# fgcallari/skeres

Measured on AMD Instinct MI355X. Metric: LM iterations/sec, higher is better.
Workload: dtype f64

## Files before the change

skeres_amd/csrc/capi.hip:

```cpp
#include <cmath>
#include <cstdlib>
#include <new>

#include "bal_kernels.hpp"
#include "dense_kernels.hpp"
#include "dense_rows_kernels.hpp"
#include "evaluate_kernels.hpp"
#include "cgnr_plan.hpp"
#include "covariance.hpp"
#include "evaluate_plan.hpp"
#include "solver.hpp"

using namespace sk;

struct sk_ptrvec { std::vector<double*> v; };
struct sk_loss_function { LossFunction l; };
struct sk_cost_function { CostFunction c; };
struct sk_problem { Problem p; };
struct sk_local_parameterization { LocalParameterization p; };
struct sk_options { Options o; };
struct sk_summary { Summary s; };
struct sk_solver { std::unique_ptr<SolverBase> impl; };
struct sk_covariance_options { CovarianceOptions o; };
struct sk_covariance { Covariance c; explicit sk_covariance(const CovarianceOptions& o) : c(o) {} };
// ... 40 lines not shown
    if (const char* e = getenv("SK_DEBUG")) {
      const std::string topics = std::string(",") + e + ",";
      k.debug_queues = topics.find(",queues,") != std::string::npos;
      k.debug_envelope = topics.find(",envelope,") != std::string::npos;
      k.debug_segments = topics.find(",segments,") != std::string::npos;
      k.debug_setup = topics.find(",setup,") != std::string::npos;
      k.debug_chain_abort = topics.find(",chain_abort,") != std::string::npos;
    }
    k.queue_shift = num("SK_QUEUE_SHIFT", 0);
    k.chain_queues = num("SK_CHAIN_QUEUES", -1);
    k.pair_max_trailing = num("SK_CHAIN_PAIR_MAX_TRAILING", 0);
    k.dissect_at = num("SK_DISSECT_AT", -1);
    k.schedule_plain = num("SK_SCHEDULE_PLAIN", 0);
    k.cgnr_batch = num("SK_CGNR_BATCH", 0);
    k.chain_xcd_local = num("SK_CHAIN_XCD_LOCAL", 0);
    if (const char* e = getenv("SK_BS_PAIR")) k.bs_pair = atoi(e);
    if (const char* e = getenv("SK_BS_SPREAD")) k.bs_spread = atoi(e);
    if (const char* e = getenv("SK_CHAIN_EARLY_SERVER")) k.chain_early_server = atoi(e);
    if (const char* e = getenv("SK_BULK_RESERVE")) {
      k.bulk_reserve = atoi(e);
      const char* c = strchr(e, ',');
      k.bulk_reserve_early = c ? atoi(c + 1) : k.bulk_reserve;
    }
    return k;
  }();
  return knobs;
}
}

extern "C" {
// ... 1186 lines not shown
```

skeres_amd/csrc/chol_kernels.hip:

```cpp
#include <hip/hip_runtime.h>
#include <algorithm>
#include <atomic>
#include <chrono>
#include <hip/hip_ext.h>
#include <math.h>
#include <stdlib.h>
#include <string.h>
#include <memory>
#include "chol_kernels.hpp"
#include "device_table.hpp"

namespace sk {

typedef double d4 __attribute__((ext_vector_type(4)));

constexpr int gemm_lds_doubles(int kBKT, int kTM, int kTN) { return 2 * (kTM + kTN) * (kBKT + 2); }
#define SK_GEMM_LDS(kBKT, kTM, kTN) __shared__ __attribute__((aligned(16))) double sh[gemm_lds_doubles(kBKT, kTM, kTN)];
template <int kMode, int kShape, int kBKT, int kPF, int kTM, int kTN>
__device__ __forceinline__ void gemm_nt_f64_body(double* shp, double* C, long ldc, const double* A, long lda, const double* B, long ldb, int K,
                                                 int tiles_m, int skip, int main_t = 0x7fffffff, int jump_t = 0, int main_n = 0x7fffffff,
                                                 int jump_n = 0, int block_id = -1, int* first_column_done = nullptr, int count_cols = 1,
                                                 int* diag_done = nullptr) {
  constexpr int mode = kMode;
  constexpr int kLdT = kBKT + 2;
// ... 376 lines not shown
#pragma unroll
    for (int nt = 0; nt < 2; ++nt)
#pragma unroll
      for (int i = 0; i < 4; ++i) acc[mt][nt][i] = sgn * src[(mt * 16 + l4 + 4 * i) * kBs + nt * 16 + l15];
}
__device__ __forceinline__ void block_update32(double* Cb, const double* P, const double* Q, int lane) {
  d4 acc[2][2];
  block_load32(acc, Cb, lane, -1.0);
  block_mma32<false>(acc, P, Q, lane);
  block_store32(Cb, acc, lane, -1.0);
}
__device__ __forceinline__ void block_to_global(double* dst, unsigned step2, unsigned goff, const double* src, int loff) {
#pragma unroll
  for (int i = 0; i < 16; ++i) dst[goff + i * step2] = src[loff + i * 2 * kBs];
}
__device__ __forceinline__ void block_neg_left_mul32(double* dst, const double* W, int lane) {
  d4 acc[2][2];
  block_zero32(acc);
  block_mma32<true>(acc, W, dst, lane);
  block_store32(dst, acc, lane, -1.0);
}

#ifdef SK_POTRF_STAMPS
__device__ long long g_potrf_stamps[4][16], g_potrf_clk[4][16];
#define SK_STAMP(i) if (lane == 0) { g_potrf_stamps[wave][i] = wall_clock64(); g_potrf_clk[wave][i] = clock64(); }
#else
#define SK_STAMP(i)
#endif

__device__ __forceinline__ void info_raise(int* info, int v) { (void)__hip_atomic_fetch_max(info, v, __ATOMIC_RELAXED, __HIP_MEMORY_SCOPE_AGENT); }

__device__ __forceinline__ void potrf128_body(double* lds_in, double* __restrict__ A, long ld, double* __restrict__ Linv, int* info) {
  double* lds = lds_in;
  int tid = threadIdx.x;
  asm volatile("" : "+v"(tid), "+s"(ld));
  double* T = lds;
  double* E = lds + 16 * kBlk;
  double* colbuf = lds + 18 * kBlk;
  volatile int* flags = reinterpret_cast<volatile int*>(colbuf + 192);
  const int t = tid, lane = t & 63, wave = __builtin_amdgcn_readfirstlane(t >> 6);
  __builtin_amdgcn_s_setprio(3);
  SK_STAMP(0)
  {
    double v0[4];
#pragma unroll
    for (int i = 0; i < 4; ++i) {
      const int e = t + 256 * i;
      v0[i] = A[(long)(e >> 5) * ld + (e & 31)];
    }
    if (wave == 0) {
#pragma unroll
      for (int i = 0; i < 4; ++i) { const int e = t + 256 * i; T[blk_off(0, 0) + (e >> 5) * kBs + (e & 31)] = v0[i]; }
      if (t < 4) flags[t] = 0;
      __syncthreads();
    } else {
      double v[3][16];
      const int first = 3 * (wave - 1) + 1;
      const long lo = (long)(lane >> 5) * ld + (lane & 31);
#pragma unroll
      for (int k = 0; k < 3; ++k) {
        const int idx = first + k, bi = idx >= 6 ? 3 : (idx >= 3 ? 2 : 1), bj = idx - bi * (bi + 1) / 2;
        const double* Ab = A + ((long)bi * kB * ld + bj * kB) + lo;
#pragma unroll
        for (int i = 0; i < 16; ++i) v[k][i] = Ab[(long)(2 * i) * ld];
      }
#pragma unroll
      for (int i = 0; i < 4; ++i) { const int e = t + 256 * i; T[blk_off(0, 0) + (e >> 5) * kBs + (e & 31)] = v0[i]; }
      __syncthreads();
// ... 26 lines not shown
    d4 xq;                                                                                       \
    quad_mma16(xq, SK_L((jb) + 1, jb), SK_L(jb, jb), qi, qj, lane, true);                        \
    __syncthreads();                                         \
    quad_store16(SK_L((jb) + 1, jb), xq, qi, qj, lane, 1.0);                                     \
    __syncthreads();                                                 \
    d4 uq;                                                                                       \
    quad_load16(uq, SK_L((jb) + 1, (jb) + 1), qi, qj, lane, -1.0);                               \
    quad_mma16(uq, SK_L((jb) + 1, jb), SK_L((jb) + 1, jb), qi, qj, lane, false);                 \
    quad_store16(SK_L((jb) + 1, (jb) + 1), uq, qi, qj, lane, -1.0);                              \
    __syncthreads();                                                                             \
  }
#define SK_WRITE_L(bi, bj) block_to_global(SK_GA(bi, bj), 2 * uld, go_a, SK_L(bi, bj), lo_w);
#define SK_WRITE_W(bi) block_to_global(SK_GI(bi, bi), 256u, go_i, SK_L(bi, bi), lo_w);
#define SK_WRITE_V(bi, bj) block_to_global(SK_GI(bi, bj), 256u, go_i, SK_V(bi, bj), lo_w);
#define SK_WRITE_E(bi) block_to_global(SK_GA(bi, bi), 2 * uld, go_a, E + ((bi) & 1) * kBlk, lo_w);
#define SK_FLAG_SET(i) { __builtin_amdgcn_fence(__ATOMIC_RELEASE, "workgroup"); __builtin_amdgcn_wave_barrier(); if (lane == 0) flags[i] = 1; }
#define SK_FLAG_WAIT(i) { while (__builtin_amdgcn_readfirstlane(flags[i]) == 0) __builtin_amdgcn_s_sleep(1); __builtin_amdgcn_fence(__ATOMIC_ACQUIRE, "workgroup"); }
  const int qi = wave >> 1, qj = wave & 1;
  if (wave == 0) {
#pragma unroll 1
    for (int jb = 0; jb < 4; ++jb) {
      double* D = SK_L(jb, jb);
      double a[32];
      const bool ok = wave_potrf32(D, colbuf, a, lane);
      SK_STAMP(11 + jb)
      if (!ok && lane == 0) info_raise(info, 1);
      {
        const int row = lane & 31;
        double* dst = lane < 32 ? E + (jb & 1) * kBlk + row * kBs : D + row;
        const int step = lane < 32 ? 1 : kBs;
// ... 6 lines not shown
      if (jb == 1) SK_CRITICAL_B(1)
      if (jb == 2) SK_CRITICAL_B(2)
      SK_STAMP(3 + 2 * jb)
    }
  } else {
    d4 accs[2][2];
    SK_STAMP(2)
    __syncthreads();
    SK_CRITICAL_B(0)
    SK_STAMP(3)
    if (wave == 1) {
      SK_PANEL_ROW(0, 2)
      SK_FLAG_SET(0)
      block_update32(SK_L(2, 2), SK_L(2, 0), SK_L(2, 0), lane);
      block_update32(SK_L(2, 1), SK_L(2, 0), SK_L(1, 0), lane);
      SK_WRITE_L(2, 0)
    }
    if (wave == 2) {
      SK_PANEL_ROW(0, 3)
      SK_FLAG_SET(1)
      block_update32(SK_L(3, 3), SK_L(3, 0), SK_L(3, 0), lane);
      block_update32(SK_L(3, 1), SK_L(3, 0), SK_L(1, 0), lane);
      SK_WRITE_L(3, 0)
    }
    if (wave == 3) {
      SK_WRITE_E(0) SK_WRITE_L(1, 0) SK_WRITE_W(0)
      SK_FLAG_WAIT(0) SK_FLAG_WAIT(1)
      block_update32(SK_L(3, 2), SK_L(3, 0), SK_L(2, 0), lane);
    }
    SK_STAMP(4)
    __syncthreads();
    SK_CRITICAL_B(1)
    SK_STAMP(5)
    if (wave == 1) {
      SK_PANEL_ROW(1, 3)
      block_update32(SK_L(3, 3), SK_L(3, 1), SK_L(3, 1), lane);
      block_update32(SK_L(3, 2), SK_L(3, 1), SK_L(2, 1), lane);
      SK_WRITE_L(3, 1) SK_WRITE_L(2, 1)
    }
    if (wave == 2) {
      d4 acc[2][2];
      block_zero32(acc);
      block_mma32<true>(acc, SK_L(1, 0), SK_L(0, 0), lane);
      block_store32(SK_V(1, 0), acc, lane, 1.0);
      block_neg_left_mul32(SK_V(1, 0), SK_L(1, 1), lane);
      SK_FLAG_SET(2)
      block_zero32(acc);
      block_mma32<true>(acc, SK_L(2, 1), SK_L(1, 1), lane);
      block_store32(SK_V(2, 1), acc, lane, 1.0);
      SK_WRITE_V(1, 0)
    }
    if (wave == 3) {
      SK_WRITE_E(1) SK_WRITE_W(1)
      block_zero32(accs);
      block_mma32<true>(accs, SK_L(2, 0), SK_L(0, 0), lane);
      SK_FLAG_WAIT(2)
      block_mma32<true>(accs, SK_L(2, 1), SK_V(1, 0), lane);
      block_store32(SK_V(2, 0), accs, lane, 1.0);
    }
    SK_STAMP(6)
    __syncthreads();
    SK_CRITICAL_B(2)
    SK_STAMP(7)
    if (wave == 1) {
      block_zero32(accs);
      block_mma32<true>(accs, SK_L(3, 0), SK_L(0, 0), lane);
      block_mma32<true>(accs, SK_L(3, 1), SK_V(1, 0), lane);
      SK_WRITE_L(3, 2)
      SK_FLAG_WAIT(3)
      block_mma32<true>(accs, SK_L(3, 2), SK_V(2, 0), lane);
      block_store32(SK_V(3, 0), accs, lane, 1.0);
      SK_WRITE_V(2, 0)
    }
    if (wave == 2) {
      block_neg_left_mul32(SK_V(2, 1), SK_L(2, 2), lane);
      block_zero32(accs);
      block_mma32<true>(accs, SK_L(3, 1), SK_L(1, 1), lane);
      block_mma32<true>(accs, SK_L(3, 2), SK_V(2, 1), lane);
      block_store32(SK_V(3, 1), accs, lane, 1.0);
      SK_WRITE_V(2, 1)
    }
    if (wave == 3) {
      block_neg_left_mul32(SK_V(2, 0), SK_L(2, 2), lane);
      SK_FLAG_SET(3)
      block_zero32(accs);
      block_mma32<true>(accs, SK_L(3, 2), SK_L(2, 2), lane);
      block_store32(SK_V(3, 2), accs, lane, 1.0);
      SK_WRITE_E(2) SK_WRITE_W(2)
    }
    SK_STAMP(8)
    __syncthreads();
  }
  if (wave < 3) {
    block_neg_left_mul32(SK_V(3, wave), SK_L(3, 3), lane);
    SK_WRITE_V(3, wave)
  } else {
    SK_WRITE_E(3) SK_WRITE_W(3)
  }
  SK_STAMP(10)
#undef SK_PANEL_ROW
#undef SK_CRITICAL_B
#undef SK_FLAG_SET
#undef SK_FLAG_WAIT
#undef SK_WRITE_L
#undef SK_WRITE_W
#undef SK_WRITE_V
#undef SK_WRITE_E
#undef SK_L
#undef SK_V
#undef SK_GA
#undef SK_GI
}

__global__ __launch_bounds__(256, 1) void potrf128_kernel(double* __restrict__ A, long ld, double* __restrict__ Linv, int* info) {
  extern __shared__ __attribute__((aligned(16))) double lds[];
  potrf128_body(lds, A, ld, Linv, info);
}
enum : int { kSyncPotrfDone = 0, kSyncAbort = 1, kSyncSyrkSeq = 2, kSyncSyrkColumn = 3, kSyncServerXcc = 4, kSyncPotrfFast = 5, kSyncStart = 6, kSyncEnd = 7,
             kSyncXSlot = 16, kSyncDSlot = 32, kSyncHeader = 64 };
constexpr int kSyncArrays = 3;
constexpr int kCritCandidates = 160;
constexpr long long kChainTimeoutTicks = 100000000;

__device__ long long g_chain_stamps[1024][8];
__device__ int g_chain_stamps_on;
#define SK_CHAIN_STAMP(col, i) if (g_chain_stamps_on && threadIdx.x == 0 && (col) < 512) g_chain_stamps[(col) + 512 * stamp_front][i] = wall_clock64();
__device__ __forceinline__ int sync_load(const int* p) { return __hip_atomic_load(p, __ATOMIC_RELAXED, __HIP_MEMORY_SCOPE_AGENT); }
__device__ __forceinline__ bool chain_wait(const int* p, int target, int* abort_flag) {
  if (sync_load(p) < target) {
    const long long t0 = wall_clock64();
    do {
      __builtin_amdgcn_s_sleep(4);
      if (sync_load(abort_flag) != 0) return false;
      if (wall_clock64() - t0 > kChainTimeoutTicks) {
        __hip_atomic_store(abort_flag, 1, __ATOMIC_RELAXED, __HIP_MEMORY_SCOPE_AGENT);
        return false;
      }
    } while (sync_load(p) < target);
  }
  __builtin_amdgcn_fence(__ATOMIC_ACQUIRE, "agent");
  asm volatile("s_waitcnt vmcnt(0)" ::: "memory");
  return true;
}
__device__ __forceinline__ bool chain_wait_start(const int* p, int value) {
  if (sync_load(p) != value) {
    const long long t0 = wall_clock64();
    int spins = 0;
    do {
      __builtin_amdgcn_s_sleep(8);
      if ((++spins & 63) == 0 && wall_clock64() - t0 > 30 * kChainTimeoutTicks) return false;
    } while (sync_load(p) != value);
  }
  __builtin_amdgcn_fence(__ATOMIC_ACQUIRE, "agent");
  asm volatile("s_waitcnt vmcnt(0)" ::: "memory");
  return true;
}
#ifdef SK_CHAIN_STRONG_FENCES
// ... 133 lines not shown
    __syncthreads();
  }
  if (local && threadIdx.x == 0) __hip_atomic_store(sync + kSyncServerXcc, 1 + xcc_id(), __ATOMIC_RELAXED, __HIP_MEMORY_SCOPE_AGENT);
  for (int r = 0; r < ranges.n; ++r)
    for (int j = ranges.begin[r]; j < ranges.end[r]; ++j) {
      if (j > 0) {
        if (threadIdx.x == 0) ok_s = server_wait_diag(sync, j, local) ? 1 : 0;
        __syncthreads();
        if (!ok_s) {
          if (threadIdx.x == 0) info_raise(info, 2);
          return;
        }
        SK_CHAIN_ACQUIRE_ALL
      }
      SK_CHAIN_STAMP(j, 0)
      potrf128_body(lds, S + (long)j * 128 * ld + (long)j * 128, ld, Linv + (long)j * 128 * 128, info);
      if (local) {
        asm volatile("s_waitcnt vmcnt(0) lgkmcnt(0)" ::: "memory");
        __syncthreads();
        if (threadIdx.x == 0) {
          store_l2(sync + kSyncPotrfFast, j + 1);
          SK_CHAIN_STAMP(j, 1)
          __builtin_amdgcn_fence(__ATOMIC_RELEASE, "agent");
          __hip_atomic_fetch_add(sync + kSyncPotrfDone, j + 1 - done, __ATOMIC_RELAXED, __HIP_MEMORY_SCOPE_AGENT);
        }
      } else {
        chain_publish(sync + kSyncPotrfDone, j + 1 - done);
        SK_CHAIN_STAMP(j, 1)
      }
      done = j + 1;
    }
// ... 42 lines not shown
  d4 acc1 = {0.0, 0.0, 0.0, 0.0};
#pragma unroll
  for (int kk = 0; kk < 32; kk += 2) {
    acc = __builtin_amdgcn_mfma_f64_16x16x4f64(sa[kk * 4], sb[kk * 4], acc, 0, 0, 0);
    acc1 = __builtin_amdgcn_mfma_f64_16x16x4f64(sa[kk * 4 + 4], sb[kk * 4 + 4], acc1, 0, 0, 0);
  }
  return acc + acc1;
}
__device__ __forceinline__ long crit_tile_off(long ldc, int i) {
  const int lane = threadIdx.x & 63, wave = threadIdx.x >> 6;
  return (long)((wave >> 1) * 16 + (lane >> 4) + 4 * i) * ldc + (wave & 1) * 16 + (lane & 15);
}

__device__ __forceinline__ void chain_column_body(int b, double* S, long ld, int j, const double* Linv_j, int tiles_m, int main_t, int jump_t,
                                                  int ncrit, double* Xs, int* sync, int maxblk, int syrk_need, int column_need, int* info, int do_next, int wait_first,
                                                  int ncand) {
  __shared__ __attribute__((aligned(16))) double sh[2 * 32 * kCritLd];
  static_assert(2 * 32 * kCritLd >= gemm_lds_doubles(16, 32, 128), "LDS of the thin tiles");
  __shared__ int ok_s;
  const int stamp_front = gridDim.y == 2 ? (int)blockIdx.y : 0;
  __builtin_amdgcn_s_setprio(2);
  double* A21 = S + (long)(j + 1) * 128 * ld + (long)j * 128;
  int* x_ready = sync + kSyncHeader + maxblk + j;
  int* diag_ready = sync + kSyncHeader + j + 1;
  int* abort_flag = sync + kSyncAbort;
  const bool local = ncand > ncrit;
  bool crit = b < ncand;
  if (crit && local) {
    if (threadIdx.x == 0) {
      int t = -1;
      if (chain_wait(sync + kSyncServerXcc, 1, abort_flag) && sync_load(sync + kSyncServerXcc) == 1 + xcc_id())
// ... 89 lines not shown
        for (int i = 0; i < 8; ++i) *reinterpret_cast<double2*>(sh + (32 + row) * kCritLd + c0 + 2 * i) = vb[i];
      }
    }
    __syncthreads();
    if (lower) {
      cacc = crit_tile_mma(sh, cacc);
#pragma unroll
      for (int i = 0; i < 4; ++i) Ct[crit_tile_off(ld, i)] = -cacc[i];
    }
    asm volatile("s_waitcnt vmcnt(0) lgkmcnt(0)" ::: "memory");
    __syncthreads();
    if (threadIdx.x == 0) store_l2(sync + kSyncDSlot + b, j + 1);
    if (stamp) SK_CHAIN_STAMP(j, 6)
    return;
  }
  if (threadIdx.x == 0)
    ok_s = (chain_wait(sync + kSyncPotrfDone, j + 1, abort_flag) &&
            (!wait_first || (chain_wait(sync + kSyncSyrkSeq, syrk_need, abort_flag) && chain_wait(sync + kSyncSyrkColumn, column_need, abort_flag)))) ? 1 : 0;
  __syncthreads();
  if (!ok_s) { if (threadIdx.x == 0) info_raise(info, 2); return; }
  SK_CHAIN_ACQUIRE_ALL
  if (stamp) SK_CHAIN_STAMP(j, 3)
  d4 xacc = {0.0, 0.0, 0.0, 0.0};
  if (crit) {
    crit_tile_load(sh, A21 + (long)ri * 32 * ld, ld, Linv_j + (long)q * 32 * 128, 128);
    __syncthreads();
    xacc = crit_tile_mma(sh, xacc);
#pragma unroll
    for (int i = 0; i < 4; ++i) store_through(Xs + (long)(ri * 32) * 128 + q * 32 + crit_tile_off(128, i), xacc[i]);
    chain_publish_through(x_ready, 1);
  } else {
    gemm_nt_f64_body<1, 0, 16, 2, 32, 128>(sh, A21, ld, A21, ld, Linv_j, 128, 128, tiles_m, 0, main_t, jump_t, 0x7fffffff, 0, thin_bid);
    asm volatile("s_waitcnt vmcnt(0) lgkmcnt(0)" ::: "memory");
    __syncthreads();
  }
  if (stamp) SK_CHAIN_STAMP(j, 4)
  if (!do_next && !crit) return;
  if (threadIdx.x == 0)
    ok_s = (chain_wait(x_ready, ncrit, abort_flag) && (!do_next || (chain_wait(sync + kSyncSyrkSeq, syrk_need, abort_flag) &&
            chain_wait(sync + kSyncSyrkColumn, column_need, abort_flag)))) ? 1 : 0;
  __syncthreads();
  if (!ok_s) { if (threadIdx.x == 0) info_raise(info, 2); return; }
  SK_CHAIN_ACQUIRE_ALL
  if (stamp) SK_CHAIN_STAMP(j, 5)
  const double* Xsrc = local ? (const double*)(Xs + (size_t)j * 128 * 128) : (const double*)Xs;
  if (crit) {
#pragma unroll
    for (int i = 0; i < 4; ++i) A21[(long)(ri * 32) * ld + q * 32 + crit_tile_off(ld, i)] = xacc[i];
    if (!do_next) return;
    if (q <= ri) {
      double* Ct = A21 + 128 + (long)(ri * 32) * ld + q * 32;
      d4 acc;
#pragma unroll
      for (int i = 0; i < 4; ++i) acc[i] = -Ct[crit_tile_off(ld, i)];
// ... 1 lines not shown
      __syncthreads();
      acc = crit_tile_mma(sh, acc);
#pragma unroll
      for (int i = 0; i < 4; ++i) store_through(Ct + crit_tile_off(ld, i), -acc[i]);
    }
    chain_publish_through(diag_ready, 1);
  } else {
    const double* Bx = ncrit ? Xsrc : (const double*)A21;
    gemm_nt_f64_body<0, 0, 16, 2, 32, 128>(sh, A21 + 128, ld, A21, ld, Bx, ncrit ? 128 : ld, 128, tiles_m, 1, main_t, jump_t, 0x7fffffff, 0, thin_bid);
    if (ncrit == 0 && b == 0) chain_publish(diag_ready, 16);
  }
  if (stamp) SK_CHAIN_STAMP(j, 6)
}
__global__ __launch_bounds__(256, 2) void chain_column_kernel(double* S, long ld, int j, const double* Linv_j, int tiles_m, int main_t, int jump_t,
                                                              int ncrit, double* Xs, int* sync, int maxblk, int syrk_need, int column_need, int* info, int do_next, int wait_first,
                                                              int ncand) {
  chain_column_body((int)blockIdx.x, S, ld, j, Linv_j, tiles_m, main_t, jump_t, ncrit, Xs, sync, maxblk, syrk_need, column_need, info, do_next, wait_first, ncand);
}
struct ColumnArgs { double* S; long ld; int j; const double* Linv_j; int tiles_m, main_t, jump_t, ncrit; double* Xs; int* sync; int maxblk, syrk_need, column_need, grid, ncand; };
struct ColumnPair { ColumnArgs f[2]; };
__global__ __launch_bounds__(256, 2) void chain_column_pair_kernel(ColumnPair pair, int* info) {
  const ColumnArgs& p = pair.f[blockIdx.y];
  if ((int)blockIdx.x >= p.grid) return;
  chain_column_body((int)blockIdx.x, p.S, p.ld, p.j, p.Linv_j, p.tiles_m, p.main_t, p.jump_t, p.ncrit, p.Xs, p.sync, p.maxblk, p.syrk_need, p.column_need, info, 1, 0, p.ncand);
}

__global__ void chain_marker_kernel(int* flag, int seq) {
  __hip_atomic_store(flag, seq, __ATOMIC_RELAXED, __HIP_MEMORY_SCOPE_AGENT);
}

__global__ __launch_bounds__(1024) void bs_step_kernel(const double* __restrict__ Linv, const double* __restrict__ Lrow, long ld,
                                                        double* __restrict__ w, double* __restrict__ yout, int kb, int col0, int ncols) {
  __shared__ double wk[128], ykb[128], part[8][128];
  const int t = threadIdx.x;
  const int c = t & 127, g = t >> 7;
  const int cl = t & 63, rg = t >> 6;
  const int col = col0 + blockIdx.x * 64 + cl;
  double wv = 0.0, li[16], lr[8];
  if (t < 128) wv = w[kb * 128 + t];
// ... 231 lines not shown
}

static const size_t g_potrf_lds = (size_t)(18 * kBlk + 192 + 4) * sizeof(double);
size_t potrf128_lds_bytes() { return g_potrf_lds; }

static std::vector<hipStream_t> g_orphan_streams;
constexpr int g_early_column = 1;
constexpr int g_thin_grid = 512;
constexpr int g_ext_events = 1;
constexpr unsigned g_event_flags = hipEventDisableTiming | hipEventDisableSystemFence;
static int g_chain_server = 1;
constexpr int g_chain_max_trailing = 24, g_chain_prefix_group = 2;
static int g_pair_max_trailing = 0;
constexpr int g_thin_syrk_tiles = 48;
constexpr int g_tail_tiles = 48, g_tail_group = 1;
static int g_chain_local = 0;
static std::atomic<int> g_bs_resident{1};
#ifdef SK_TESTING
static std::atomic<int> g_test_withhold{-1};
static std::atomic<int> g_test_janitor_giveup{0};
#endif
hipError_t cholesky_init() {
  static std::once_flag once;
  std::call_once(once, [] {
#ifdef SK_TESTING
    if (const char* e = getenv("SK_CHAIN_TEST_WITHHOLD_MARKER")) g_test_withhold.store(atoi(e));
    if (const char* e = getenv("SK_BS_TEST_JANITOR_GIVEUP")) g_test_janitor_giveup.store(atoi(e) > 0 ? 1 : 0);
#endif
    const DevKnobs& k = dev_knobs();
    g_bs_resident.store(k.bs_resident);
    g_chain_server = k.chain_server;
    g_pair_max_trailing = k.pair_max_trailing;
    g_chain_local = k.chain_xcd_local;
  });
  hipError_t rc = hipFuncSetAttribute(reinterpret_cast<const void*>(potrf_server_kernel), hipFuncAttributeMaxDynamicSharedMemorySize, (int)g_potrf_lds);
  if (rc != hipSuccess) return rc;
  rc = hipFuncSetAttribute(reinterpret_cast<const void*>(potrf_server_pair_kernel), hipFuncAttributeMaxDynamicSharedMemorySize, (int)g_potrf_lds);
  if (rc != hipSuccess) return rc;
  return hipFuncSetAttribute(reinterpret_cast<const void*>(potrf128_kernel), hipFuncAttributeMaxDynamicSharedMemorySize, 160 * 1024);
}

CholeskyContext::~CholeskyContext() {
  for (hipEvent_t e : events) (void)hipEventDestroy(e);
  if (fork_ev) (void)hipEventDestroy(fork_ev);
  if (join_ev) (void)hipEventDestroy(join_ev);
  if (sync) (void)hipFree(sync);
  if (xs) (void)hipFree(xs);
}
// ... 522 lines not shown
  ChainRanges ranges;
  ranges.n = 0;
  for (int j = 0; j < nblk; ++j)
    if (plan.resident[j] && (j == 0 || !plan.resident[j - 1])) {
      if (ranges.n == 8) { ranges.n = 0; break; }
      int e = j;
      while (e < nblk && plan.resident[e]) ++e;
      ranges.begin[ranges.n] = j; ranges.end[ranges.n] = e; ++ranges.n;
    }
  bool chain = ranges.n > 0 && ctx->dq && ctx->dq->chain_server && ctx->resident && !(kt && kt->times_all());
  int* sync = chain ? ctx->sync_for(nblk) : nullptr;
  if (!sync) chain = false;
  auto is_resident = [&](int k) { return chain && k < nblk && plan.resident[k]; };
  const int local = chain && (g_chain_local == 1 || (g_chain_local == 2 && !(partner && partner->ncols > 0))) ? 1 : 0;
  auto column_grid = [&](int ncrit, int T, int ncand) { return ncrit ? ncand + 4 * T - 4 : 4 * T; };
  const int maxblk = chain ? ctx->sync_blk : 0;
  const char* stamps_file = chain ? dev_knobs().chain_stamps : nullptr;
  hipStream_t srv = nullptr;
  hipEvent_t start_ev = nullptr;
  int start_value = 0;
  struct PartnerState {
    bool on = false; CholeskyPlan plan; int nblk = 0, ncols = 0, tail0 = 0, start_at = 0, maxblk = 0; const int* last = nullptr; const int* tail = nullptr;
    double* S = nullptr; long ld = 0; double* Linv = nullptr; int* sync = nullptr; double* xs = nullptr;
    int next = 0, seq = 0, col_seq = 0;
  } pb;
  struct PartnerStep { ColumnArgs col; ThinSyrkArgs syrk; int Tb; bool next_resident, by_column; };
  auto partner_step = [&](int kB) {
    PartnerStep st;
    auto lm = [&](int c) { return pb.last ? (pb.last[c] < pb.nblk - 1 ? pb.last[c] : pb.nblk - 1) : pb.nblk - 1; };
    auto rf = [&](int first_row, int last_row) {
      Rows r;
      r.main = last_row >= first_row ? last_row - first_row + 1 : 0;
      const int t0 = std::max(pb.tail ? pb.tail[kB] : pb.tail0, first_row + r.main);
      r.extra = std::max(0, pb.nblk - t0);
      r.jump = r.extra ? t0 - (first_row + r.main) : 0;
      return r;
    };
    const int k1 = kB + 1, Lg = lm(kB);
    const Rows rn = rf(k1, Lg), rs = rf(k1 + 1, Lg);
    const int T = rn.main + rn.extra, ncrit = (rn.main > 0 || rn.jump == 0) ? 16 : 0;
    st.Tb = rs.main + rs.extra;
    st.next_resident = k1 < pb.ncols;
    st.by_column = st.next_resident && g_early_column;
    const int ncand = ncrit && local ? kCritCandidates : ncrit;
    st.col = ColumnArgs{pb.S, pb.ld, kB, pb.Linv + (long)kB * 128 * 128, 4 * T, 4 * rn.main, 4 * rn.jump, ncrit, pb.xs, pb.sync, pb.maxblk, pb.seq, pb.col_seq,
                        column_grid(ncrit, T, ncand), ncand};
    st.syrk = ThinSyrkArgs{pb.S + (long)(k1 + 1) * 128 * pb.ld + (long)(k1 + 1) * 128, pb.ld, pb.S + (long)(k1 + 1) * 128 * pb.ld + (long)kB * 128, pb.ld, 128, 4 * st.Tb,
                           4 * rs.main, 4 * rs.jump, rs.main, rs.jump, st.by_column ? pb.sync + kSyncSyrkColumn : (int*)nullptr, st.Tb > 0 ? 2 * st.Tb * (st.Tb + 1) : 0};
    return st;
  };
  auto partner_advance = [&](const PartnerStep& st, hipStream_t bulk_stream) {
    if (st.Tb > 0) {
      if (st.by_column) pb.col_seq += 4 * st.Tb;
      else if (st.next_resident) { ++pb.seq; hipLaunchKernelGGL(chain_marker_kernel, dim3(1), dim3(1), 0, bulk_stream, pb.sync + kSyncSyrkSeq, pb.seq); }
    }
    ++pb.next;
  };
  if (chain) {
    const int stamps_on = stamps_file ? 1 : 0;
    static int stamps_state = 0;
    if (stamps_on != stamps_state) { (void)hipMemcpyToSymbol(HIP_SYMBOL(g_chain_stamps_on), &stamps_on, sizeof(int)); stamps_state = stamps_on; }
// ... 66 lines not shown
    const double* P = S + (long)k1 * 128 * ld + (long)k0 * 128;
    const int Tb = rs.main + rs.extra;
    if (la) sb = Tb >= ctx->early_tiles ? ctx->bulk_early : ctx->bulk;
    if (la && Tb > 0 && sb == ctx->bulk_early) used_bulk_early = true;
    if (sb != sb_prev && syrk_done) (void)hipStreamWaitEvent(sb, syrk_done, 0);
    sb_prev = sb;
    if (resident && pair) {
      if (syrk_done2) (void)hipStreamWaitEvent(sp, syrk_done2, 0);
      hipEvent_t col_done = ctx->event(ev++);
      for (int c = 0; c < 2; ++c) {
        const Rows rc = rows_from(k0 + c + 1, k0 + c);
        const int T = rc.main + rc.extra;
        const int ncrit = (rc.main > 0 || rc.jump == 0) ? 16 : 0;
        hipExtLaunchKernelGGL(chain_column_kernel, dim3(ncrit ? 16 + 4 * T - 4 : 4 * T), dim3(256), 0, sp, nullptr, c == 1 ? col_done : (hipEvent_t) nullptr, 0, S, ld,
                              k0 + c, (const double*)(Linv + (long)(k0 + c) * 128 * 128), 4 * T, 4 * rc.main, 4 * rc.jump, ncrit, ctx->xs, sync, maxblk, seq, col_seq, info,
                              c == 0 ? 1 : 0, c == 0 && after_pair ? 1 : 0, ncrit);
      }
      (void)hipStreamWaitEvent(sb, col_done, 0);
    } else if (resident) {
      const int T = rn.main + rn.extra;
      const int ncrit = (rn.main > 0 || rn.jump == 0) ? 16 : 0;
      const int ncand = ncrit && local && !after_pair ? kCritCandidates : ncrit;
      with_partner = pb.on && k0 >= pb.start_at && pb.next < pb.ncols && !after_pair && Tb <= g_thin_syrk_tiles && ctx->early_tiles > g_thin_syrk_tiles;
      if (with_partner) pst = partner_step(pb.next);
      hipEvent_t col_done = (Tb > 0 || (with_partner && pst.Tb > 0)) ? ctx->event(ev++) : nullptr;
      if (with_partner) {
        ColumnPair cp;
        cp.f[0] = ColumnArgs{S, ld, k0, Linv + (long)k0 * 128 * 128, 4 * T, 4 * rn.main, 4 * rn.jump, ncrit, ctx->xs, sync, maxblk, seq, col_seq, column_grid(ncrit, T, ncand), ncand};
        cp.f[1] = pst.col;
        hipExtLaunchKernelGGL(chain_column_pair_kernel, dim3(std::max(cp.f[0].grid, cp.f[1].grid), 2), dim3(256), 0, sp, nullptr, col_done, 0, cp, info);
      } else {
        hipExtLaunchKernelGGL(chain_column_kernel, dim3(column_grid(ncrit, T, ncand)), dim3(256), 0, sp, nullptr, col_done, 0, S, ld, k0,
                              (const double*)(Linv + (long)k0 * 128 * 128), 4 * T, 4 * rn.main, 4 * rn.jump, ncrit, ctx->xs, sync, maxblk, seq, col_seq, info, 1, after_pair ? 1 : 0, ncand);
      }
      if (col_done) (void)hipStreamWaitEvent(sb, col_done, 0);
    } else {
      if (panel_done) (void)hipStreamWaitEvent(sb, panel_done, 0);
      else order(sp, sb);
      if (la && syrk_done) (void)hipStreamWaitEvent(sp, syrk_done, 0);
      update(sp, "gemm_syrk_next", A22, P, P, K, rn, na, 1);
    }
    syrk_done = nullptr;
    if (with_partner) {
      const bool by_col = next_resident && g_early_column;
      bool withheld = false;
#ifdef SK_TESTING
      if (next_resident && Tb > 0 && !ctx->dq->tuning) { int want = k1; withheld = want >= 0 && g_test_withhold.compare_exchange_strong(want, -1); }
#endif
// ... 87 lines not shown
  order(sp, s);
  if (la) { order(ctx->bulk, s); if (used_bulk_early) order(ctx->bulk_early, s); }
  if (chain) order(srv, s);
  }
  if (stamps_file) {
    (void)hipStreamSynchronize(s);
    std::vector<long long> st((size_t)1024 * 8);
    (void)hipMemcpyFromSymbol(st.data(), HIP_SYMBOL(g_chain_stamps), st.size() * sizeof(long long));
    const std::string stamps_name = std::string(stamps_file) + (partner && partner->ncols > 0 ? ".pair" : "");
    if (FILE* f = fopen(stamps_name.c_str(), "w")) {
      for (int j = 0; j < nblk && j < 512; ++j) {
        if (!plan.resident[j]) continue;
        fprintf(f, "%d ", j);
        for (int i = 0; i < 7; ++i) fprintf(f, "%lld ", st[(size_t)j * 8 + i]);
        const Rows rs = rows_from(j + 2, j);
        fprintf(f, "%d\n", rs.main + rs.extra);
      }
      for (int j = 0; partner && j < partner->ncols && j < 512; ++j) {
        fprintf(f, "%d ", 512 + j);
        for (int i = 0; i < 7; ++i) fprintf(f, "%lld ", st[(size_t)(512 + j) * 8 + i]);
        fprintf(f, "0\n");
      }
      fclose(f);
    }
  }
}

bool cholesky_backsolve_resident(int nblk) { return g_bs_resident.load() != 0 && nblk <= kBsMaxBlocks; }
static int bs_janitors(int owners) { return std::max(1, std::min(owners, 96)); }
void cholesky_backsolve(double* S, long ld, int n, int npad, int rhs_row, const double* Linv, double* w, double* y,
                        hipStream_t s, KernelTimer* kt, const int* last, int* info, const int* tail, bool zero_after, int resident, bool prefilled) {
  const int nblk = npad / 128;
  if (info && (resident < 0 ? g_bs_resident.load() != 0 : resident != 0) && nblk <= kBsMaxBlocks) {
    BsTop env;
    for (int c = 0; c < nblk; ++c) {
      env.top[c] = (unsigned short)(last ? std::min(std::max(last[c], c), nblk - 1) : nblk - 1);
// ... 279 lines not shown
```

skeres_amd/csrc/dev_knobs.hpp:

```cpp
#pragma once

namespace sk {

struct DevKnobs {
  int chain_server = 1;
  int bs_resident = 1;
  const char* chain_stamps = nullptr;
  const char* bs_stamps = nullptr;
  bool debug_queues = false, debug_envelope = false, debug_segments = false, debug_chain_abort = false, debug_setup = false;
  int queue_shift = 0;
  int chain_queues = -1;
  int pair_max_trailing = 0;
  int dissect_at = -1;
  int chain_early_server = 1;
  int bs_spread = 1;
  int bs_pair = 1;
  int bulk_reserve = -1, bulk_reserve_early = -1;
  int chain_xcd_local = 0;
  int cgnr_batch = 0;
  int schedule_plain = 0;
};
const DevKnobs& dev_knobs();

}
```

Before: 259.4.

## Stage POTRF panel publication so critical column tiles start on partial factors

The 128-block POTRF now writes each 32-column panel of L and its inverse diagonal through to global memory and publishes a per-stage counter. Critical column blocks in the chain kernel wait on these stage counters and run the triangular solve and diagonal update one 32-slice at a time, instead of waiting for the whole POTRF to finish. The aim is to overlap the column TRSM/SYRK with the tail of the diagonal factorization on the critical path. This adds more fine-grained spin-waits, atomic write-through stores and LDS reloading, which raises complexity and synchronization overhead.

```diff
diff --git a/skeres_amd/csrc/capi.hip b/skeres_amd/csrc/capi.hip
--- a/skeres_amd/csrc/capi.hip
+++ b/skeres_amd/csrc/capi.hip
@@ -78,6 +78,7 @@
     k.schedule_plain = num("SK_SCHEDULE_PLAIN", 0);
     k.cgnr_batch = num("SK_CGNR_BATCH", 0);
     k.chain_xcd_local = num("SK_CHAIN_XCD_LOCAL", 0);
+    k.chain_staged = num("SK_CHAIN_STAGED", 1);
     if (const char* e = getenv("SK_BS_PAIR")) k.bs_pair = atoi(e);
     if (const char* e = getenv("SK_BS_SPREAD")) k.bs_spread = atoi(e);
     if (const char* e = getenv("SK_CHAIN_EARLY_SERVER")) k.chain_early_server = atoi(e);
diff --git a/skeres_amd/csrc/chol_kernels.hip b/skeres_amd/csrc/chol_kernels.hip
--- a/skeres_amd/csrc/chol_kernels.hip
+++ b/skeres_amd/csrc/chol_kernels.hip
@@ -414,6 +414,10 @@
 #pragma unroll
   for (int i = 0; i < 16; ++i) dst[goff + i * step2] = src[loff + i * 2 * kBs];
 }
+__device__ __forceinline__ void block_to_global_through(double* dst, unsigned step2, unsigned goff, const double* src, int loff) {
+#pragma unroll
+  for (int i = 0; i < 16; ++i) __hip_atomic_store(dst + (goff + i * step2), src[loff + i * 2 * kBs], __ATOMIC_RELAXED, __HIP_MEMORY_SCOPE_AGENT);
+}
 __device__ __forceinline__ void block_neg_left_mul32(double* dst, const double* W, int lane) {
   d4 acc[2][2];
   block_zero32(acc);
@@ -430,7 +434,7 @@
 
 __device__ __forceinline__ void info_raise(int* info, int v) { (void)__hip_atomic_fetch_max(info, v, __ATOMIC_RELAXED, __HIP_MEMORY_SCOPE_AGENT); }
 
-__device__ __forceinline__ void potrf128_body(double* lds_in, double* __restrict__ A, long ld, double* __restrict__ Linv, int* info) {
+__device__ __forceinline__ void potrf128_body(double* lds_in, double* __restrict__ A, long ld, double* __restrict__ Linv, int* info, int* stage = nullptr, int stage_base = 0) {
   double* lds = lds_in;
   int tid = threadIdx.x;
   asm volatile("" : "+v"(tid), "+s"(ld));
@@ -451,7 +455,7 @@
     if (wave == 0) {
 #pragma unroll
       for (int i = 0; i < 4; ++i) { const int e = t + 256 * i; T[blk_off(0, 0) + (e >> 5) * kBs + (e & 31)] = v0[i]; }
-      if (t < 4) flags[t] = 0;
+      if (t < 5) flags[t] = 0;
       __syncthreads();
     } else {
       double v[3][16];
@@ -508,6 +512,13 @@
 #define SK_WRITE_W(bi) block_to_global(SK_GI(bi, bi), 256u, go_i, SK_L(bi, bi), lo_w);
 #define SK_WRITE_V(bi, bj) block_to_global(SK_GI(bi, bj), 256u, go_i, SK_V(bi, bj), lo_w);
 #define SK_WRITE_E(bi) block_to_global(SK_GA(bi, bi), 2 * uld, go_a, E + ((bi) & 1) * kBlk, lo_w);
+#define SK_STAGE_L(bi, bj) { if (stage) block_to_global_through(SK_GA(bi, bj), 2 * uld, go_a, SK_L(bi, bj), lo_w); else SK_WRITE_L(bi, bj) }
+#define SK_STAGE_W(bi) { if (stage) block_to_global_through(SK_GI(bi, bi), 256u, go_i, SK_L(bi, bi), lo_w); else SK_WRITE_W(bi) }
+#define SK_STAGE_PUBLISH(t)                                                                                               \
+  if (stage) {                                                                                                           \
+    asm volatile("s_waitcnt vmcnt(0)" ::: "memory");    \
+    if (lane == 0) __hip_atomic_store(stage, stage_base + (t) + 1, __ATOMIC_RELAXED, __HIP_MEMORY_SCOPE_AGENT);           \
+  }
 #define SK_FLAG_SET(i) { __builtin_amdgcn_fence(__ATOMIC_RELEASE, "workgroup"); __builtin_amdgcn_wave_barrier(); if (lane == 0) flags[i] = 1; }
 #define SK_FLAG_WAIT(i) { while (__builtin_amdgcn_readfirstlane(flags[i]) == 0) __builtin_amdgcn_s_sleep(1); __builtin_amdgcn_fence(__ATOMIC_ACQUIRE, "workgroup"); }
   const int qi = wave >> 1, qj = wave & 1;
@@ -544,19 +555,19 @@
       SK_FLAG_SET(0)
       block_update32(SK_L(2, 2), SK_L(2, 0), SK_L(2, 0), lane);
       block_update32(SK_L(2, 1), SK_L(2, 0), SK_L(1, 0), lane);
-      SK_WRITE_L(2, 0)
     }
     if (wave == 2) {
       SK_PANEL_ROW(0, 3)
       SK_FLAG_SET(1)
       block_update32(SK_L(3, 3), SK_L(3, 0), SK_L(3, 0), lane);
       block_update32(SK_L(3, 1), SK_L(3, 0), SK_L(1, 0), lane);
-      SK_WRITE_L(3, 0)
     }
     if (wave == 3) {
-      SK_WRITE_E(0) SK_WRITE_L(1, 0) SK_WRITE_W(0)
+      SK_STAGE_W(0) SK_STAGE_L(1, 0) SK_WRITE_E(0)
       SK_FLAG_WAIT(0) SK_FLAG_WAIT(1)
+      SK_STAGE_L(2, 0) SK_STAGE_L(3, 0)
       block_update32(SK_L(3, 2), SK_L(3, 0), SK_L(2, 0), lane);
+      SK_STAGE_PUBLISH(0)
     }
     SK_STAMP(4)
     __syncthreads();
@@ -564,9 +575,9 @@
     SK_STAMP(5)
     if (wave == 1) {
       SK_PANEL_ROW(1, 3)
+      SK_FLAG_SET(4)
       block_update32(SK_L(3, 3), SK_L(3, 1), SK_L(3, 1), lane);
       block_update32(SK_L(3, 2), SK_L(3, 1), SK_L(2, 1), lane);
-      SK_WRITE_L(3, 1) SK_WRITE_L(2, 1)
     }
     if (wave == 2) {
       d4 acc[2][2];
@@ -581,12 +592,15 @@
       SK_WRITE_V(1, 0)
     }
     if (wave == 3) {
-      SK_WRITE_E(1) SK_WRITE_W(1)
+      SK_STAGE_W(1) SK_STAGE_L(2, 1) SK_WRITE_E(1)
       block_zero32(accs);
       block_mma32<true>(accs, SK_L(2, 0), SK_L(0, 0), lane);
+      SK_FLAG_WAIT(4)
+      SK_STAGE_L(3, 1)
       SK_FLAG_WAIT(2)
       block_mma32<true>(accs, SK_L(2, 1), SK_V(1, 0), lane);
       block_store32(SK_V(2, 0), accs, lane, 1.0);
+      SK_STAGE_PUBLISH(1)
     }
     SK_STAMP(6)
     __syncthreads();
@@ -596,7 +610,6 @@
       block_zero32(accs);
       block_mma32<true>(accs, SK_L(3, 0), SK_L(0, 0), lane);
       block_mma32<true>(accs, SK_L(3, 1), SK_V(1, 0), lane);
-      SK_WRITE_L(3, 2)
       SK_FLAG_WAIT(3)
       block_mma32<true>(accs, SK_L(3, 2), SK_V(2, 0), lane);
       block_store32(SK_V(3, 0), accs, lane, 1.0);
@@ -611,12 +624,14 @@
       SK_WRITE_V(2, 1)
     }
     if (wave == 3) {
+      SK_STAGE_W(2) SK_STAGE_L(3, 2)
       block_neg_left_mul32(SK_V(2, 0), SK_L(2, 2), lane);
       SK_FLAG_SET(3)
+      SK_STAGE_PUBLISH(2)
       block_zero32(accs);
       block_mma32<true>(accs, SK_L(3, 2), SK_L(2, 2), lane);
       block_store32(SK_V(3, 2), accs, lane, 1.0);
-      SK_WRITE_E(2) SK_WRITE_W(2)
+      SK_WRITE_E(2)
     }
     SK_STAMP(8)
     __syncthreads();
@@ -625,7 +640,9 @@
     block_neg_left_mul32(SK_V(3, wave), SK_L(3, 3), lane);
     SK_WRITE_V(3, wave)
   } else {
-    SK_WRITE_E(3) SK_WRITE_W(3)
+    SK_STAGE_W(3)
+    SK_STAGE_PUBLISH(3)
+    SK_WRITE_E(3)
   }
   SK_STAMP(10)
 #undef SK_PANEL_ROW
@@ -636,6 +653,9 @@
 #undef SK_WRITE_W
 #undef SK_WRITE_V
 #undef SK_WRITE_E
+#undef SK_STAGE_L
+#undef SK_STAGE_W
+#undef SK_STAGE_PUBLISH
 #undef SK_L
 #undef SK_V
 #undef SK_GA
@@ -647,7 +667,7 @@
   potrf128_body(lds, A, ld, Linv, info);
 }
 enum : int { kSyncPotrfDone = 0, kSyncAbort = 1, kSyncSyrkSeq = 2, kSyncSyrkColumn = 3, kSyncServerXcc = 4, kSyncPotrfFast = 5, kSyncStart = 6, kSyncEnd = 7,
-             kSyncXSlot = 16, kSyncDSlot = 32, kSyncHeader = 64 };
+             kSyncXSlot = 16, kSyncDSlot = 32, kSyncStage = 48, kSyncHeader = 64 };
 constexpr int kSyncArrays = 3;
 constexpr int kCritCandidates = 160;
 constexpr long long kChainTimeoutTicks = 100000000;
@@ -671,6 +691,40 @@
   __builtin_amdgcn_fence(__ATOMIC_ACQUIRE, "agent");
   asm volatile("s_waitcnt vmcnt(0)" ::: "memory");
   return true;
+}
+__device__ __forceinline__ int chain_wait_value(const int* p, int target, int* abort_flag) {
+  int v = sync_load(p);
+  if (v < target) {
+    const long long t0 = wall_clock64();
+    for (;;) {
+      __builtin_amdgcn_s_sleep(1);
+      const int a = sync_load(abort_flag);
+      v = sync_load(p);
+      if (v >= target) break;
+      if (a != 0) return -1;
+      if (wall_clock64() - t0 > kChainTimeoutTicks) {
+        __hip_atomic_store(abort_flag, 1, __ATOMIC_RELAXED, __HIP_MEMORY_SCOPE_AGENT);
+        return -1;
+      }
+    }
+  }
+  __builtin_amdgcn_fence(__ATOMIC_ACQUIRE, "agent");
+  asm volatile("s_waitcnt vmcnt(0)" ::: "memory");
+  return v;
+}
+__device__ __forceinline__ bool chain_wait_pair_nofence(const int* p0, int need0, const int* p1, int need1, int* abort_flag) {
+  if (sync_load(p0) >= need0 && sync_load(p1) >= need1) return true;
+  const long long t0 = wall_clock64();
+  for (;;) {
+    __builtin_amdgcn_s_sleep(2);
+    const int a = sync_load(abort_flag), v0 = sync_load(p0), v1 = sync_load(p1);
+    if (v0 >= need0 && v1 >= need1) return true;
+    if (a != 0) return false;
+    if (wall_clock64() - t0 > kChainTimeoutTicks) {
+      __hip_atomic_store(abort_flag, 1, __ATOMIC_RELAXED, __HIP_MEMORY_SCOPE_AGENT);
+      return false;
+    }
+  }
 }
 __device__ __forceinline__ bool chain_wait_start(const int* p, int value) {
   if (sync_load(p) != value) {
@@ -834,7 +888,7 @@
         SK_CHAIN_ACQUIRE_ALL
       }
       SK_CHAIN_STAMP(j, 0)
-      potrf128_body(lds, S + (long)j * 128 * ld + (long)j * 128, ld, Linv + (long)j * 128 * 128, info);
+      potrf128_body(lds, S + (long)j * 128 * ld + (long)j * 128, ld, Linv + (long)j * 128 * 128, info, local ? (int*)nullptr : sync + kSyncStage, 4 * j);
       if (local) {
         asm volatile("s_waitcnt vmcnt(0) lgkmcnt(0)" ::: "memory");
         __syncthreads();
@@ -907,7 +961,7 @@
 
 __device__ __forceinline__ void chain_column_body(int b, double* S, long ld, int j, const double* Linv_j, int tiles_m, int main_t, int jump_t,
                                                   int ncrit, double* Xs, int* sync, int maxblk, int syrk_need, int column_need, int* info, int do_next, int wait_first,
-                                                  int ncand) {
+                                                  int ncand, int staged) {
   __shared__ __attribute__((aligned(16))) double sh[2 * 32 * kCritLd];
   static_assert(2 * 32 * kCritLd >= gemm_lds_doubles(16, 32, 128), "LDS of the thin tiles");
   __shared__ int ok_s;
@@ -1027,6 +1081,119 @@
     if (stamp) SK_CHAIN_STAMP(j, 6)
     return;
   }
+  if (crit && staged) {
+    int* rows_loaded = sync + kSyncHeader + 2 * maxblk + j;
+    if (q > ri) {
+      if (threadIdx.x == 0) __hip_atomic_fetch_add(diag_ready, 1, __ATOMIC_RELAXED, __HIP_MEMORY_SCOPE_AGENT);
+      return;
+    }
+    const int lane = threadIdx.x & 63, wave = threadIdx.x >> 6, l15 = lane & 15, l4 = lane >> 4, qi = wave >> 1, qj = wave & 1;
+    const double* Ljj = A21 - (long)128 * ld;
+    double* Ct = A21 + 128 + (long)(ri * 32) * ld + q * 32;
+    crit_tile_load(sh, A21 + (long)ri * 32 * ld, ld, A21 + (long)q * 32 * ld, ld);
+    __syncthreads();
+    if (threadIdx.x == 0) __hip_atomic_fetch_add(rows_loaded, (1 << (8 * ri)) + (q != ri ? 1 << (8 * q) : 0), __ATOMIC_RELAXED, __HIP_MEMORY_SCOPE_AGENT);
+    double* za = sh + (qi * 16 + l15) * kCritLd + l4;
+    double* zc = sh + (qi * 16 + l4) * kCritLd + qj * 16 + l15;
+    const double* zb = sh + (32 + qj * 16 + l15) * kCritLd + l4;
+    d4 dacc = {0.0, 0.0, 0.0, 0.0};
+    d4 x3 = {0.0, 0.0, 0.0, 0.0}, cld = {0.0, 0.0, 0.0, 0.0};
+    double w[4][8], lf[6][8];
+    __shared__ int have_s, syrk_ok_s;
+    int have = 0;
+#pragma unroll
+    for (int t = 0; t < 4; ++t) {
+      const bool look = have <= t;
+      if (t > 0) __syncthreads();
+      if (look || t == 3) {
+        if (look && threadIdx.x == 0) have_s = chain_wait_value(sync + kSyncStage, 4 * j + t + 1, abort_flag);
+        if (t == 3 && threadIdx.x == 64) syrk_ok_s = chain_wait_pair_nofence(sync + kSyncSyrkSeq, syrk_need, sync + kSyncSyrkColumn, column_need, abort_flag) ? 1 : 0;
+        __syncthreads();
+        if ((look && have_s < 0) || (t == 3 && !syrk_ok_s)) { if (threadIdx.x == 0) info_raise(info, 2); return; }
+        SK_CHAIN_ACQUIRE_ALL
+        if (t == 3) {
+#pragma unroll
+          for (int i = 0; i < 4; ++i) cld[i] = __hip_atomic_load(Ct + crit_tile_off(ld, i), __ATOMIC_RELAXED, __HIP_MEMORY_SCOPE_AGENT);
+        }
+        if (look) {
+          const int now = have_s - 4 * j < 4 ? have_s - 4 * j : 4;
+#pragma unroll
+          for (int s = t; s < 4; ++s)
+            if (s < now) {
+              if (stamp) SK_CHAIN_STAMP(j, s < 3 ? 3 + s : 7)
+#pragma unroll
+              for (int kk = 0; kk < 8; ++kk) w[s][kk] = Linv_j[(long)(s * 32 + qj * 16 + l15) * 128 + s * 32 + kk * 4 + l4];
+#pragma unroll
+              for (int u = s + 1; u < 4; ++u)
+#pragma unroll
+                for (int kk = 0; kk < 8; ++kk) lf[s * (7 - s) / 2 + u - s - 1][kk] = Ljj[(long)(u * 32 + qj * 16 + l15) * ld + s * 32 + kk * 4 + l4];
+            }
+          have = now;
+        }
+      }
+      d4 x[2];
+#pragma unroll
+      for (int sl = 0; sl < 2; ++sl) {
+        x[sl] = (d4){0.0, 0.0, 0.0, 0.0};
+#pragma unroll
+        for (int kk = 0; kk < 8; ++kk) x[sl] = __builtin_amdgcn_mfma_f64_16x16x4f64(za[sl * 32 * kCritLd + t * 32 + kk * 4], w[t][kk], x[sl], 0, 0, 0);
+      }
+      __syncthreads();
+#pragma unroll
+      for (int sl = 0; sl < 2; ++sl)
+#pragma unroll
+        for (int i = 0; i < 4; ++i) zc[(sl * 32 + 4 * i) * kCritLd + t * 32] = x[sl][i];
+      if (ri == q && t < 3) {
+#pragma unroll
+        for (int i = 0; i < 4; ++i) store_through(Xs + (long)(ri * 32) * 128 + t * 32 + crit_tile_off(128, i), x[0][i]);
+      }
+      if (t == 3) { x3 = x[0]; dacc -= cld; }
+      __syncthreads();
+#pragma unroll
+      for (int u = t + 1; u < 4; ++u)
+#pragma unroll
+        for (int sl = 0; sl < 2; ++sl) {
+          d4 z;
+#pragma unroll
+          for (int i = 0; i < 4; ++i) z[i] = -zc[(sl * 32 + 4 * i) * kCritLd + u * 32];
+#pragma unroll
+          for (int kk = 0; kk < 8; ++kk) z = __builtin_amdgcn_mfma_f64_16x16x4f64(za[sl * 32 * kCritLd + t * 32 + kk * 4], lf[t * (7 - t) / 2 + u - t - 1][kk], z, 0, 0, 0);
+#pragma unroll
+          for (int i = 0; i < 4; ++i) zc[(sl * 32 + 4 * i) * kCritLd + u * 32] = -z[i];
+        }
+#pragma unroll
+      for (int kk = 0; kk < 8; ++kk) dacc = __builtin_amdgcn_mfma_f64_16x16x4f64(za[t * 32 + kk * 4], zb[t * 32 + kk * 4], dacc, 0, 0, 0);
+    }
+#pragma unroll
+    for (int i = 0; i < 4; ++i) store_through(Ct + crit_tile_off(ld, i), -dacc[i]);
+    chain_publish_through(diag_ready, 1);
+    if (stamp) SK_CHAIN_STAMP(j, 6)
+    if (ri == q) {
+#pragma unroll
+      for (int i = 0; i < 4; ++i) store_through(Xs + (long)(ri * 32) * 128 + 96 + crit_tile_off(128, i), x3[i]);
+      chain_publish_through(x_ready, 1);
+    }
+    if (ri == 3) {
+      if (threadIdx.x == 0) {
+        bool ok = true;
+        if (((sync_load(rows_loaded) >> (8 * q)) & 0xff) < 4) {
+          const long long t0 = wall_clock64();
+          do {
+            __builtin_amdgcn_s_sleep(4);
+            if (sync_load(abort_flag) != 0 || wall_clock64() - t0 > kChainTimeoutTicks) { __hip_atomic_store(abort_flag, 1, __ATOMIC_RELAXED, __HIP_MEMORY_SCOPE_AGENT); ok = false; break; }
+          } while (((sync_load(rows_loaded) >> (8 * q)) & 0xff) < 4);
+        }
+        ok_s = ok ? 1 : 0;
+      }
+      __syncthreads();
+      if (!ok_s) { if (threadIdx.x == 0) info_raise(info, 2); return; }
+      const int t = threadIdx.x, row = t >> 3, c0 = (t & 7) * 16;
+#pragma unroll
+      for (int i = 0; i < 8; ++i)
+        *reinterpret_cast<double2*>(A21 + (long)(q * 32 + row) * ld + c0 + 2 * i) = *reinterpret_cast<const double2*>(sh + (32 + row) * kCritLd + c0 + 2 * i);
+    }
+    return;
+  }
   if (threadIdx.x == 0)
     ok_s = (chain_wait(sync + kSyncPotrfDone, j + 1, abort_flag) &&
             (!wait_first || (chain_wait(sync + kSyncSyrkSeq, syrk_need, abort_flag) && chain_wait(sync + kSyncSyrkColumn, column_need, abort_flag)))) ? 1 : 0;
@@ -1050,7 +1217,7 @@
   if (stamp) SK_CHAIN_STAMP(j, 4)
   if (!do_next && !crit) return;
   if (threadIdx.x == 0)
-    ok_s = (chain_wait(x_ready, ncrit, abort_flag) && (!do_next || (chain_wait(sync + kSyncSyrkSeq, syrk_need, abort_flag) &&
+    ok_s = (chain_wait(x_ready, staged ? 4 : ncrit, abort_flag) && (!do_next || (chain_wait(sync + kSyncSyrkSeq, syrk_need, abort_flag) &&
             chain_wait(sync + kSyncSyrkColumn, column_need, abort_flag)))) ? 1 : 0;
   __syncthreads();
   if (!ok_s) { if (threadIdx.x == 0) info_raise(info, 2); return; }
@@ -1082,15 +1249,15 @@
 }
 __global__ __launch_bounds__(256, 2) void chain_column_kernel(double* S, long ld, int j, const double* Linv_j, int tiles_m, int main_t, int jump_t,
                                                               int ncrit, double* Xs, int* sync, int maxblk, int syrk_need, int column_need, int* info, int do_next, int wait_first,
-                                                              int ncand) {
-  chain_column_body((int)blockIdx.x, S, ld, j, Linv_j, tiles_m, main_t, jump_t, ncrit, Xs, sync, maxblk, syrk_need, column_need, info, do_next, wait_first, ncand);
-}
-struct ColumnArgs { double* S; long ld; int j; const double* Linv_j; int tiles_m, main_t, jump_t, ncrit; double* Xs; int* sync; int maxblk, syrk_need, column_need, grid, ncand; };
+                                                              int ncand, int staged) {
+  chain_column_body((int)blockIdx.x, S, ld, j, Linv_j, tiles_m, main_t, jump_t, ncrit, Xs, sync, maxblk, syrk_need, column_need, info, do_next, wait_first, ncand, staged);
+}
+struct ColumnArgs { double* S; long ld; int j; const double* Linv_j; int tiles_m, main_t, jump_t, ncrit; double* Xs; int* sync; int maxblk, syrk_need, column_need, grid, ncand, staged; };
 struct ColumnPair { ColumnArgs f[2]; };
 __global__ __launch_bounds__(256, 2) void chain_column_pair_kernel(ColumnPair pair, int* info) {
   const ColumnArgs& p = pair.f[blockIdx.y];
   if ((int)blockIdx.x >= p.grid) return;
-  chain_column_body((int)blockIdx.x, p.S, p.ld, p.j, p.Linv_j, p.tiles_m, p.main_t, p.jump_t, p.ncrit, p.Xs, p.sync, p.maxblk, p.syrk_need, p.column_need, info, 1, 0, p.ncand);
+  chain_column_body((int)blockIdx.x, p.S, p.ld, p.j, p.Linv_j, p.tiles_m, p.main_t, p.jump_t, p.ncrit, p.Xs, p.sync, p.maxblk, p.syrk_need, p.column_need, info, 1, 0, p.ncand, p.staged);
 }
 
 __global__ void chain_marker_kernel(int* flag, int seq) {
@@ -1352,6 +1519,7 @@
 static int g_pair_max_trailing = 0;
 constexpr int g_thin_syrk_tiles = 48;
 constexpr int g_tail_tiles = 48, g_tail_group = 1;
+static int g_chain_staged = 1;
 static int g_chain_local = 0;
 static std::atomic<int> g_bs_resident{1};
 #ifdef SK_TESTING
@@ -1370,6 +1538,7 @@
     g_chain_server = k.chain_server;
     g_pair_max_trailing = k.pair_max_trailing;
     g_chain_local = k.chain_xcd_local;
+    g_chain_staged = k.chain_staged;
   });
   hipError_t rc = hipFuncSetAttribute(reinterpret_cast<const void*>(potrf_server_kernel), hipFuncAttributeMaxDynamicSharedMemorySize, (int)g_potrf_lds);
   if (rc != hipSuccess) return rc;
@@ -1922,6 +2091,7 @@
   auto is_resident = [&](int k) { return chain && k < nblk && plan.resident[k]; };
   const int local = chain && (g_chain_local == 1 || (g_chain_local == 2 && !(partner && partner->ncols > 0))) ? 1 : 0;
   auto column_grid = [&](int ncrit, int T, int ncand) { return ncrit ? ncand + 4 * T - 4 : 4 * T; };
+  auto column_staged = [&](int ncrit, int ncand, bool shared) { return g_chain_staged >= (shared ? 2 : 1) && ncrit == 16 && ncand == ncrit ? 1 : 0; };
   const int maxblk = chain ? ctx->sync_blk : 0;
   const char* stamps_file = chain ? dev_knobs().chain_stamps : nullptr;
   hipStream_t srv = nullptr;
@@ -1952,7 +2122,7 @@
     st.by_column = st.next_resident && g_early_column;
     const int ncand = ncrit && local ? kCritCandidates : ncrit;
     st.col = ColumnArgs{pb.S, pb.ld, kB, pb.Linv + (long)kB * 128 * 128, 4 * T, 4 * rn.main, 4 * rn.jump, ncrit, pb.xs, pb.sync, pb.maxblk, pb.seq, pb.col_seq,
-                        column_grid(ncrit, T, ncand), ncand};
+                        column_grid(ncrit, T, ncand), ncand, column_staged(ncrit, ncand, true)};
     st.syrk = ThinSyrkArgs{pb.S + (long)(k1 + 1) * 128 * pb.ld + (long)(k1 + 1) * 128, pb.ld, pb.S + (long)(k1 + 1) * 128 * pb.ld + (long)kB * 128, pb.ld, 128, 4 * st.Tb,
                            4 * rs.main, 4 * rs.jump, rs.main, rs.jump, st.by_column ? pb.sync + kSyncSyrkColumn : (int*)nullptr, st.Tb > 0 ? 2 * st.Tb * (st.Tb + 1) : 0};
     return st;
@@ -2049,7 +2219,7 @@
         const int ncrit = (rc.main > 0 || rc.jump == 0) ? 16 : 0;
         hipExtLaunchKernelGGL(chain_column_kernel, dim3(ncrit ? 16 + 4 * T - 4 : 4 * T), dim3(256), 0, sp, nullptr, c == 1 ? col_done : (hipEvent_t) nullptr, 0, S, ld,
                               k0 + c, (const double*)(Linv + (long)(k0 + c) * 128 * 128), 4 * T, 4 * rc.main, 4 * rc.jump, ncrit, ctx->xs, sync, maxblk, seq, col_seq, info,
-                              c == 0 ? 1 : 0, c == 0 && after_pair ? 1 : 0, ncrit);
+                              c == 0 ? 1 : 0, c == 0 && after_pair ? 1 : 0, ncrit, 0);
       }
       (void)hipStreamWaitEvent(sb, col_done, 0);
     } else if (resident) {
@@ -2061,12 +2231,12 @@
       hipEvent_t col_done = (Tb > 0 || (with_partner && pst.Tb > 0)) ? ctx->event(ev++) : nullptr;
       if (with_partner) {
         ColumnPair cp;
-        cp.f[0] = ColumnArgs{S, ld, k0, Linv + (long)k0 * 128 * 128, 4 * T, 4 * rn.main, 4 * rn.jump, ncrit, ctx->xs, sync, maxblk, seq, col_seq, column_grid(ncrit, T, ncand), ncand};
+        cp.f[0] = ColumnArgs{S, ld, k0, Linv + (long)k0 * 128 * 128, 4 * T, 4 * rn.main, 4 * rn.jump, ncrit, ctx->xs, sync, maxblk, seq, col_seq, column_grid(ncrit, T, ncand), ncand, column_staged(ncrit, ncand, true)};
         cp.f[1] = pst.col;
         hipExtLaunchKernelGGL(chain_column_pair_kernel, dim3(std::max(cp.f[0].grid, cp.f[1].grid), 2), dim3(256), 0, sp, nullptr, col_done, 0, cp, info);
       } else {
         hipExtLaunchKernelGGL(chain_column_kernel, dim3(column_grid(ncrit, T, ncand)), dim3(256), 0, sp, nullptr, col_done, 0, S, ld, k0,
-                              (const double*)(Linv + (long)k0 * 128 * 128), 4 * T, 4 * rn.main, 4 * rn.jump, ncrit, ctx->xs, sync, maxblk, seq, col_seq, info, 1, after_pair ? 1 : 0, ncand);
+                              (const double*)(Linv + (long)k0 * 128 * 128), 4 * T, 4 * rn.main, 4 * rn.jump, ncrit, ctx->xs, sync, maxblk, seq, col_seq, info, 1, after_pair ? 1 : 0, ncand, after_pair ? 0 : column_staged(ncrit, ncand, false));
       }
       if (col_done) (void)hipStreamWaitEvent(sb, col_done, 0);
     } else {
@@ -2184,12 +2354,12 @@
         fprintf(f, "%d ", j);
         for (int i = 0; i < 7; ++i) fprintf(f, "%lld ", st[(size_t)j * 8 + i]);
         const Rows rs = rows_from(j + 2, j);
-        fprintf(f, "%d\n", rs.main + rs.extra);
+        fprintf(f, "%d %lld\n", rs.main + rs.extra, st[(size_t)j * 8 + 7]);
       }
       for (int j = 0; partner && j < partner->ncols && j < 512; ++j) {
         fprintf(f, "%d ", 512 + j);
         for (int i = 0; i < 7; ++i) fprintf(f, "%lld ", st[(size_t)(512 + j) * 8 + i]);
-        fprintf(f, "0\n");
+        fprintf(f, "0 %lld\n", st[(size_t)(512 + j) * 8 + 7]);
       }
       fclose(f);
     }
diff --git a/skeres_amd/csrc/dev_knobs.hpp b/skeres_amd/csrc/dev_knobs.hpp
--- a/skeres_amd/csrc/dev_knobs.hpp
+++ b/skeres_amd/csrc/dev_knobs.hpp
@@ -17,6 +17,7 @@
   int bs_pair = 1;
   int bulk_reserve = -1, bulk_reserve_early = -1;
   int chain_xcd_local = 0;
+  int chain_staged = 1;
   int cgnr_batch = 0;
   int schedule_plain = 0;
 };
```

Result: slower. 255.9 (-1.3%).
